# jianwen-xie/Latent-Space-Normalizing-Flow

Measured on AMD Instinct MI355X. Metric: latent-samples/sec through flow+logdet, nz=128 B=65536, higher is better.
Workload: dtype bf16x3; 1 GPU; CIFAR-10 flow prior nz=128 f_width=64 f_depth=5 affine, forward+logdet+log-prob, B=65536 synthetic z per evaluation (BASELINE.json configs[2]); rows_per_gpu=65536, global_rows=65536, parallelism=single GPU, streams=3, clock_ramp_launches_before_warmup=600

## Files before the change

### latent-space-normalizing-flow_amd/csrc/lsnf_device.h

```cpp
#pragma once
#include <hip/hip_runtime.h>
#include <type_traits>
#include "lsnf_layout.h"

typedef float f32x16 __attribute__((ext_vector_type(16)));
typedef float f32x4 __attribute__((ext_vector_type(4)));

#define LSNF_WG_THREADS 256
#define LSNF_WG_WAVES 4
#define LSNF_WG_SAMPLES (LSNF_WG_WAVES * 32)

#define LSNF_AS1 __attribute__((address_space(1)))
#define LSNF_AS3 __attribute__((address_space(3)))

static inline hipError_t lsnf_allow_big_lds(const void* kernel, unsigned long long* done_mask) {
    int dev = 0;
    hipError_t e = hipGetDevice(&dev);
    if (e != hipSuccess) return e;
    if (dev >= 0 && dev < 64 && ((*done_mask >> dev) & 1ull)) return hipSuccess;
    e = hipFuncSetAttribute(kernel, hipFuncAttributeMaxDynamicSharedMemorySize, 160 * 1024);
    if (e != hipSuccess) return e;
    if (dev >= 0 && dev < 64) *done_mask |= 1ull << dev;
    return hipSuccess;
}
// ... 25 lines not shown
    static constexpr int OFF_S4 = OFF_S3 + LSNF_FRAG_FLOATS * P3 * KT3;
    static constexpr int FWD_BLOCK = OFF_S4 + LSNF_FRAG_FLOATS * P4 * KT4;
    static constexpr int FWD_CONST = 32 * NP + 32;
    static constexpr int INV_BLOCK = LSNF_FRAG_FLOATS * NZT * NZT;
    static constexpr int INV_CONST = 32 * NZT;
    static constexpr int OFF_B4 = 0;
    static constexpr int OFF_B3 = OFF_B4 + LSNF_FRAG_FLOATS * WT * 2 * HT;
    static constexpr int OFF_B2 = OFF_B3 + LSNF_FRAG_FLOATS * WT * WT;
    static constexpr int OFF_B1 = OFF_B2 + LSNF_FRAG_FLOATS * HT * WT;
    static constexpr int BWD_BLOCK = OFF_B1 + LSNF_FRAG_FLOATS * NZT * NZT;
    static constexpr int MAXKT = (NZT > WT ? NZT : WT);
    static constexpr int SLOT = 2 * MAXKT * LSNF_FRAG_FLOATS;
};

#define LSNF_STATS_SLOTS 64
__device__ __forceinline__ void lsnf_publish_stats(double* stats, double sum_ll, double sum_logdet, int rows, int lane) {
    const unsigned grid = gridDim.x, wg = blockIdx.x;
    unsigned long long* ticket = reinterpret_cast<unsigned long long*>(&stats[2]);
    int last = 0;
    if (lane == 0) {
        const unsigned s = wg % LSNF_STATS_SLOTS;
        double* sub = stats + 8 + 4 * s;
        const double r0 = atomicAdd(&sub[0], sum_ll);
        const double r1 = atomicAdd(&sub[1], sum_logdet);
        unsigned long long inc = 1ull;
        asm volatile("" : "+v"(inc) : "v"(r0), "v"(r1));
        bool slot_done = true;
        if (grid > LSNF_STATS_SLOTS) {
            const unsigned long long n_s = (grid - s + LSNF_STATS_SLOTS - 1) / LSNF_STATS_SLOTS;
            unsigned long long* st = reinterpret_cast<unsigned long long*>(&sub[2]);
            slot_done = atomicAdd(st, inc) == n_s - 1;
            if (slot_done) atomicExch(st, 0ull);
            inc = 1ull;
        }
        if (slot_done) {
            const unsigned long long slots = grid > LSNF_STATS_SLOTS ? LSNF_STATS_SLOTS : grid;
            if (atomicAdd(ticket, inc) == slots - 1) { last = 1; atomicExch(ticket, 0ull); }
// ... 24 lines not shown
        if (PIECES % NW == 0 || seg < PIECES) {
            const float* g = gsrc + seg * 256 + lane * 4;
            float* l = lbuf + seg * 256;
            __builtin_amdgcn_global_load_lds((const LSNF_AS1 void*)g, (LSNF_AS3 void*)l, 16, 0, 0);
        }
    }
}

__device__ __forceinline__ void lsnf_panel_barrier() {
    asm volatile("s_waitcnt vmcnt(0)" ::: "memory");
#ifndef LSNF_ABLATE_BARRIER
    __syncthreads();
#endif
}

template <int KT>
__device__ __forceinline__ void lsnf_panel_mma(f32x16& acc, const f32x16* in, const float* lbuf, int lane) {
    const f32x4* wp = reinterpret_cast<const f32x4*>(lbuf) + lane;
    __builtin_amdgcn_sched_barrier(0);
    f32x4 w0 = wp[0], w1 = wp[64], w2 = wp[128], w3 = wp[192];
    __builtin_amdgcn_sched_group_barrier(0x100, 4, 0);
#pragma unroll
    for (int kt = 0; kt < KT; ++kt) {
        f32x4 n0 = w0, n1 = w1, n2 = w2, n3 = w3;
        if (kt + 1 < KT) {
            n0 = wp[((kt + 1) * 4 + 0) * 64]; n1 = wp[((kt + 1) * 4 + 1) * 64];
            n2 = wp[((kt + 1) * 4 + 2) * 64]; n3 = wp[((kt + 1) * 4 + 3) * 64];
        }
#define LSNF_MFMA4(W, G)                                                                      \
        acc = __builtin_amdgcn_mfma_f32_32x32x2f32(W[0], in[kt][4 * G + 0], acc, 0, 0, 0);    \
// ... 14 lines not shown
#pragma unroll
    for (int q = 0; q < 4; ++q) {
        const f32x4 v = b[q];
        a[4 * q + 0] = v[0]; a[4 * q + 1] = v[1]; a[4 * q + 2] = v[2]; a[4 * q + 3] = v[3];
    }
    return a;
}

__device__ __forceinline__ f32x16 lsnf_zero16() {
    f32x16 a;
#pragma unroll
    for (int r = 0; r < 16; ++r) a[r] = 0.0f;
    return a;
}

__device__ __forceinline__ f32x16 lsnf_relu16(f32x16 a) {
#pragma unroll
    for (int r = 0; r < 16; ++r) a[r] = fmaxf(a[r], 0.0f);
    return a;
}

__device__ __forceinline__ void lsnf_sigmoid_log2(float p, float& sig, float& l2) {
    const float pc = __builtin_amdgcn_fmed3f(p, -80.0f, 80.0f);
    const float e = __builtin_amdgcn_exp2f(pc * -1.4426950408889634f);
    const float d = 1.0f + e;
    sig = __builtin_amdgcn_rcpf(d);
    l2 = __builtin_amdgcn_logf(d);
}

__device__ __forceinline__ void lsnf_sigmoid_logsig(float p, float& sig, float& lsig) {
#ifdef LSNF_ABLATE_EPILOGUE
    sig = p * 0.25f + 0.5f; lsig = p; return;
#endif
// ... 251 lines not shown
```

### latent-space-normalizing-flow_amd/csrc/lsnf_fwd.hip

```cpp
#include <stdlib.h>
#include "lsnf_device.h"

namespace {

template <int HT_, int WT_>
struct FwdCfg : LsnfStackCfg<HT_, WT_> {
    using B = LsnfStackCfg<HT_, WT_>;
    static constexpr int BLOCK_FLOATS = B::FWD_BLOCK, CONST_FLOATS = B::FWD_CONST;
};

struct FwdArgs {
    const float* consts;
    const float* panels;
    const float* z_in;
    const float* objective;
    float* z_out;
    float* logdet_out;
    float* ll_out;
    float* z_saved;
    float* act_saved;
    int B, nz, half, n_blocks, vec4;
    double* stats;
    unsigned long long* stamps;
};
// ... 19 lines not shown
    constexpr int FWD_THREADS = 64 * FWD_WAVES;
    constexpr int HT = C::HT, WT = C::WT, NZT = C::NZT;
    extern __shared__ __attribute__((aligned(16))) float smem[];
    float* cst = smem;
    float* buf0 = smem + a.n_blocks * C::CONST_FLOATS;
    const int tid = threadIdx.x;
    const int wave = __builtin_amdgcn_readfirstlane(tid >> 6);
    const int lane = tid & 63;
    const int m = lane & 31, h = lane >> 5;

    LSNF_STAMP(0);
    LSNF_STAMP_RT(50);
    LsnfPipeT<FWD_WAVES> pipe;
    pipe.buf0 = buf0; pipe.slot = C::SLOT; pipe.wave = wave; pipe.lane = lane;
    pipe.template prime<lsnf_first_ktc(C::P1, C::KT1)>(a.panels);
    for (int i = tid; i < a.n_blocks * C::CONST_FLOATS; i += FWD_THREADS) cst[i] = a.consts[i];

    const long sample = ((long)blockIdx.x * FWD_WAVES + wave) * 32 + m;
    const bool live = sample < a.B;
    const long row = live ? sample : (long)a.B - 1;

    f32x16 x[NZT];
#ifdef LSNF_ABLATE_IO
#pragma unroll
    for (int t = 0; t < NZT; ++t)
#pragma unroll
        for (int r = 0; r < 16; ++r) x[t][r] = 0.001f * (float)(lane + r + t);
    float ell = 0.0f;
#else
    lsnf_load_rows<HT>(x, a.z_in, row, a.nz, a.half, h, a.vec4);
    float ell = a.objective ? a.objective[row] : 0.0f;
// ... 80 lines not shown
    if (live) {
        {
            float* zo = a.z_out + sample * (long)a.nz;
#pragma unroll
            for (int t = HT; t < NZT; ++t) lsnf_store_tile<HT>(t, x[t], zo, a.half, h, a.vec4);
        }
        if (h == 0) {
            a.logdet_out[sample] = ell;
            if (a.ll_out) a.ll_out[sample] = (-0.5f * ss + 1.8378770664093453f) + ell;
        }
    }
    if (a.stats) {
        float sl = (live && h == 0) ? ((-0.5f * ss + 1.8378770664093453f) + ell) : 0.0f;
        float sd = (live && h == 0) ? ell : 0.0f;
        double dl = (double)sl, dd = (double)sd;
#pragma unroll
        for (int o = 16; o > 0; o >>= 1) { dl += __shfl_xor(dl, o, 64); dd += __shfl_xor(dd, o, 64); }
        __syncthreads();
        double* red = reinterpret_cast<double*>(buf0);
        if (lane == 0) { red[2 * wave] = dl; red[2 * wave + 1] = dd; }
        __syncthreads();
        if (wave == 0) {
            double tl = 0.0, td = 0.0;
            for (int w = 0; w < FWD_WAVES; ++w) { tl += red[2 * w]; td += red[2 * w + 1]; }
            lsnf_publish_stats(a.stats, tl, td, a.B, lane);
        }
    }
    LSNF_STAMP(40);
    asm volatile("s_waitcnt vmcnt(0)" ::: "memory");
    LSNF_STAMP(41);
    LSNF_STAMP_RT(51);
}
// ... 40 lines not shown
```

### latent-space-normalizing-flow_amd/csrc/lsnf_fwd3.hip

```cpp
#include <stdlib.h>
#include "lsnf_l16.h"

namespace {



template <int HT_, int WT_>
struct Fwd3Cfg : LsnfStackCfg<HT_, WT_> {
    using S = LsnfStackCfg<HT_, WT_>;
    static constexpr int F = L16_FRAG_FLOATS;
    static constexpr int OFF3_S2 = F * S::P1 * S::KT1;
    static constexpr int OFF3_S3 = OFF3_S2 + F * S::P2 * S::KT2;
    static constexpr int OFF3_S4 = OFF3_S3 + F * S::P3 * S::KT3;
    static constexpr int BLOCK3 = OFF3_S4 + F * S::P4 * S::KT4;
    static constexpr int SLOT3 = 2 * S::MAXKT * F;
    static constexpr int CONST_FLOATS = S::FWD_CONST;
};

struct Fwd3Args {
    const float* consts; const float* panels3;
    const float* z_in; const float* objective;
    float* z_out; float* logdet_out; float* ll_out; float* z_saved; float* act_saved;
    int B, nz, half, n_blocks, vec4;
    double* stats;
// ... 49 lines not shown
    }
    bool bad = false;
#endif
    Pipe3<F3_WAVES> pipe;
    pipe.buf0 = buf0; pipe.slot = C::SLOT3; pipe.wave = wave; pipe.lane = lane;
    pipe.template prime<first_kib(C::P1, C::KT1)>(a.panels3);

    int sample[2], rows[2]; bool live[2];
#pragma unroll
    for (int st = 0; st < 2; ++st) { sample[st] = wbase + 16 * st + n; live[st] = sample[st] < a.B; rows[st] = live[st] ? sample[st] : a.B - 1; }

    f32x16 x[NZT];
#pragma unroll
    for (int t = 0; t < NZT; ++t) x[t] = l16_load_tile<HT>(t, a.z_in, rows, a.nz, a.half, g, a.vec4);
    __builtin_amdgcn_sched_barrier(0);
    for (int i = tid; i < a.n_blocks * C::CONST_FLOATS; i += THREADS) cst[i] = a.consts[i];
    float ell[2];
#pragma unroll
    for (int st = 0; st < 2; ++st) ell[st] = a.objective ? a.objective[rows[st]] : 0.0f;

    const LsnfActLayout al = lsnf_act_layout(a.B, HT, WT);
    const LsnfDumpLayout dl = lsnf_dump_layout(a.B, a.nz, a.width);
    const bool w4 = (a.width & 3) == 0;
    const size_t wtile = (size_t)blockIdx.x * F3_WAVES + wave;
    for (int blk = 0; blk < a.n_blocks; ++blk) {
        float* act = (a.act_saved && wtile * 32 < (size_t)a.B)
                         ? a.act_saved + (size_t)blk * al.per_block + wtile * al.per_tile : nullptr;
        const float* cb = cst + blk * C::CONST_FLOATS;
        const float* gblk = a.panels3 + (size_t)blk * C::BLOCK3;
        const bool more = blk + 1 < a.n_blocks;
        const float* gnext = more ? gblk + C::BLOCK3 : nullptr;
// ... 119 lines not shown
            int smp = sample[st];
            asm volatile("" : "+v"(smp));
            float ld = ell[st];
#if LSNF_L16_PARTS == 2
            if (wave_bad && st == 0 && n == 0) ld = __builtin_bit_cast(float, LSNF_F16_SENTINEL_BITS);
#endif
            a.logdet_out[smp] = ld;
            if (a.ll_out) a.ll_out[smp] = ll[st];
        }
    }
    if (a.stats) {
        double dl = 0.0, dd = 0.0;
#pragma unroll
        for (int st = 0; st < 2; ++st)
            if (live[st] && g == 0) { dl += (double)ll[st]; dd += (double)ell[st]; }
#pragma unroll
        for (int o = 8; o > 0; o >>= 1) { dl += __shfl_xor(dl, o, 64); dd += __shfl_xor(dd, o, 64); }
        __syncthreads();
        double* red = reinterpret_cast<double*>(buf0);
        if (lane == 0) { red[2 * wave] = dl; red[2 * wave + 1] = dd; }
        __syncthreads();
        if (wave == 0) {
            double tl = 0.0, td = 0.0;
            for (int w = 0; w < F3_WAVES; ++w) { tl += red[2 * w]; td += red[2 * w + 1]; }
            lsnf_publish_stats(a.stats, tl, td, a.B, lane);
        }
    }
    F3_STAMP(41, "s_memtime");
    F3_STAMP(51, "s_memrealtime");
}

template <class C>
// ... 58 lines not shown
```

### latent-space-normalizing-flow_amd/csrc/lsnf_fwd3p.hip

```cpp
#include <stdlib.h>
#include <type_traits>
#include "lsnf_l16.h"

#if LSNF_L16_PARTS != 3
#error "lsnf_fwd3p.hip is the three-term bf16 kernel"
#endif

#ifndef LSNF_FILLMASK
#define LSNF_FILLMASK 0x7f
#endif

namespace {

struct Fwd3pArgs {
    const float* consts; const float* panels3;
    const float* z_in; const float* objective;
    float* z_out; float* logdet_out; float* ll_out;
    int B, nz, half, n_blocks, vec4;
    double* stats;
    float* hdump; int width;
    float* z_saved; float* act_saved;
    unsigned long long* stamps;
};

// ... 5 lines not shown
         if (a.stamps && lane == 0) a.stamps[(((size_t)blockIdx.x * NWAVES + wave) & 2047) * 64 + (i)] = t_; } while (0)
#else
#define P_STAMP(i, INSN) do {} while (0)
#endif

template <int WT_>
struct Fwd3pCfg : LsnfStackCfg<2, WT_> {
    using S = LsnfStackCfg<2, WT_>;
    static constexpr int F = LSNF_FRAG3_FLOATS;
    static constexpr int OFF3_S2 = F * S::P1 * S::KT1;
    static constexpr int OFF3_S3 = OFF3_S2 + F * S::P2 * S::KT2;
    static constexpr int OFF3_S4 = OFF3_S3 + F * S::P3 * S::KT3;
    static constexpr int BLOCK3 = OFF3_S4 + F * S::P4 * S::KT4;
    static constexpr int SLOT3 = 2 * S::MAXKT * F;
    static constexpr int CONST_FLOATS = S::FWD_CONST;
};

__device__ __forceinline__ void keep(unsigned a, unsigned b, unsigned c) { asm volatile("" :: "v"(a), "v"(b), "v"(c)); }
__device__ __forceinline__ void keep(float a, float b, float c, float d, float e) { asm volatile("" :: "v"(a), "v"(b), "v"(c), "v"(d), "v"(e)); }

struct StepDesc { int acc, tile, s, frag; };
template <int KT> constexpr StepDesc mkstep(int acc, int tl, int in_tile, int kt, int s) { return StepDesc{acc, in_tile, s, ((tl * KT + kt) * 2 + s) * 3}; }

struct Tile16 { f32x4v q[4]; };
struct SplitTile16 { unsigned d[2][3][4]; };

template <int HT, int ST>
__device__ __forceinline__ Tile16 load_tile16(int t, const float* __restrict__ z, const int* rows, int nz, int half, int g, int vw) {
    Tile16 x;
    const int hh = t / HT, tt = t % HT;
// ... 54 lines not shown
    for (int j = 0; j < i; ++j)
        if (PH::at(j).acc == PH::at(i).acc && PH::at(j).s == PH::at(i).s) return false;
    return true;
}
template <int ST> __device__ __forceinline__ constexpr int unit_quad(int q) { return ST == 2 ? q : (q & ~1); }
template <int ST> __device__ __forceinline__ constexpr int unit_pair0(int q) { return ST == 2 ? 0 : (q & 1); }
template <int ST> __device__ __forceinline__ constexpr int unit_st(int q) { return ST == 2 ? (q & 1) : 0; }
template <bool RELU, int ST>
__device__ __forceinline__ void split_q16(const Tile16& x, int q, SplitTile16& out) {
#pragma clang fp contract(off)
    const int ft = q >> 1, st = unit_st<ST>(q), qr = unit_quad<ST>(q);
#pragma unroll
    for (int jj = 0; jj < ST; ++jj) {
        const int j = unit_pair0<ST>(q) + jj;
        float a = x.q[qr][2 * j], b = x.q[qr][2 * j + 1];
        if (RELU) { a = fmaxf(a, 0.0f); b = fmaxf(b, 0.0f); }
        const unsigned p1 = pk_bf16(a, b);
        a -= __builtin_bit_cast(float, p1 << 16); b -= __builtin_bit_cast(float, p1 & 0xffff0000u);
        const unsigned p2 = pk_bf16(a, b);
        a -= __builtin_bit_cast(float, p2 << 16); b -= __builtin_bit_cast(float, p2 & 0xffff0000u);
        const int d = 2 * ft + j;
        out.d[st][0][d] = p1; out.d[st][1][d] = p2; out.d[st][2][d] = pk_bf16(a, b);
        keep(out.d[st][0][d], out.d[st][1][d], out.d[st][2][d]);
    }
}
template <int ST>
__device__ __forceinline__ void sigmoid_q16(Tile16& p, int q, float* lsum ) {
    const int st = unit_st<ST>(q), qr = unit_quad<ST>(q), r0 = 2 * unit_pair0<ST>(q);
#pragma unroll
    for (int r = r0; r < r0 + 2 * ST; ++r) {
        float sig, l2;
// ... 31 lines not shown
    if (st) off += (unsigned)(16 * nz * 4);
    off = (32 * tt + 16 * ft + 4 * g < half) ? off : 0x80000000u;
    const u32x4s v = __builtin_bit_cast(u32x4s, x.q[q]);
    __builtin_amdgcn_raw_buffer_store_b128(v, rs.r[hh], off + (unsigned)((32 * tt + 16 * ft) * 4), 0, LSNF_STASH_AUX);
}
__device__ __forceinline__ void stash_sigma_quad(const StashRsrc& rs, const StashLane& sl, int t, int q, const Tile16& sg) {
    if constexpr (!(LSNF_STASH_PARTS & 2)) return;
    const int ft = q >> 1, st = q & 1;
    const u32x4s v = __builtin_bit_cast(u32x4s, sg.q[q]);
    __builtin_amdgcn_raw_buffer_store_b128(v, rs.r[t], sl.soff + (unsigned)((2 * ft * 64 + 16 * st) * 16), 0, LSNF_STASH_AUX);
}
__device__ __forceinline__ void mask_q16(const Tile16& h, int q, unsigned (&mk)[2][2]) {
    if constexpr (!(LSNF_STASH_PARTS & 1)) return;
    unsigned m = 0;
#pragma unroll
    for (int r = 3; r >= 0; --r) m = __builtin_amdgcn_alignbit(m, __builtin_bit_cast(unsigned, 0.0f - h.q[q][r]), 31);
    mk[q & 1][q >> 1] = m;
    asm volatile("" :: "v"(m));
}
__device__ __forceinline__ void stash_mask_words(const StashRsrc& rs, const StashLane& sl, int tile, const unsigned (&mk)[2][2]) {
    if constexpr (!(LSNF_STASH_PARTS & 1)) return;
    const unsigned w0 = mk[0][0] | (mk[0][1] << 8), w1 = mk[1][0] | (mk[1][1] << 8);
    unsigned x = ((w0 << 16) | w1) << sl.msh;
    x = lsnf_pair_or32(x);
    __builtin_amdgcn_raw_buffer_store_b32(x >> 16, rs.r[0], sl.moff + (unsigned)(tile * 64 * 4), 0, 0);
    __builtin_amdgcn_raw_buffer_store_b32(x & 0xffffu, rs.r[0], sl.moff + (unsigned)((tile * 64 + 16) * 4), 0, 0);
}
__device__ __forceinline__ void stash_h_quad(const StashRsrc& rs, const StashLane& sl, int t, int q, const Tile16& h, int width) {
    const int ft = q >> 1, st = q & 1;
    f32x4v r;
#pragma unroll
    for (int j = 0; j < 4; ++j) r[j] = fmaxf(h.q[q][j], 0.0f);
    const unsigned off = (32 * t + 16 * ft < width) ? sl.hoff : 0x80000000u;
    __builtin_amdgcn_raw_buffer_store_b128(__builtin_bit_cast(u32x4s, r), rs.r[t], off + (unsigned)((ft * 2 + st) * 1024), 0, LSNF_STASH_AUX);
}

template <int NM, int NV>
__device__ __forceinline__ void pin_mfma() {
    lsnf_static_for<NM>([&](auto mc) {
        constexpr int m = decltype(mc)::value, V = NV / NM + (m < NV % NM ? 1 : 0);
        __builtin_amdgcn_sched_group_barrier(0x008, 1, 0);
        if constexpr (V > 0) __builtin_amdgcn_sched_group_barrier(0x402, V, 0);
    });
}
template <class PH, int ST, class Fill, class Mid>
__device__ __forceinline__ void run_phase16(Tile16* acc, const float* bias_ptr , const SplitTile16* in, const float* lbuf, int lane, Fill&& fill, Mid&& mid) {
    const bf16x8* wp = reinterpret_cast<const bf16x8*>(lbuf) + lane;
// ... 119 lines not shown
    const int wave = __builtin_amdgcn_readfirstlane(tid >> 6);
    const int lane = tid & 63;
    const int n = lane & 15, g = lane >> 4;
    P_STAMP(0, "s_memtime");
    P_STAMP(50, "s_memrealtime");
    const int n_phases = 4 * a.n_blocks;
    auto phase_src = [&](int k) -> const float* {
        const float* gb = a.panels3 + (size_t)(k >> 2) * C::BLOCK3;
        const int j = k & 3;
        return gb + (j == 0 ? 0 : (j == 1 ? 2 * 4 * F : (j == 2 ? C::OFF3_S2 : C::OFF3_S4)));
    };
    auto sync_issue = [&](int k, auto left) {
#ifdef LSNF_ABL_SKIPSYNC
        if ((LSNF_ABL_SKIPSYNC >> (k & 3)) & 1) return;
#endif
        asm volatile("s_waitcnt vmcnt(%0)" :: "n"(decltype(left)::value) : "memory");
        __syncthreads();
#ifdef LSNF_FWD3Q_BURST_DMA
        if (k + 1 < n_phases) issue_kib<48, NWAVES>(phase_src(k + 1), buf0 + ((k + 1) & 1) * SLOT, wave, lane);
#endif
    };
    constexpr int PER_WAVE = 48 / NWAVES, EVERY = STASH ? 1 : 16 / PER_WAVE, LAST_DMA = (PER_WAVE - 1) * EVERY;
    using Left0 = std::integral_constant<int, 0>;
    using LeftS1a = std::integral_constant<int, stores_after<TS1a>(LAST_DMA)>;
    using LeftS1b = std::integral_constant<int, stores_after<TS1b>(LAST_DMA)>;
    using LeftS23 = std::integral_constant<int, stores_after<TS23>(LAST_DMA) + (STASH == 2 ? 1 : 0)>;
    using LeftS4 = std::integral_constant<int, stores_after<TS4>(LAST_DMA)>;
    const float* dma_src = nullptr; float* dma_dst = nullptr;
    auto dma_arm = [&](int k) {
        dma_src = phase_src(k + 1 < n_phases ? k + 1 : k);
        dma_dst = buf0 + ((k + 1) & 1) * SLOT;
    };
    auto dma_step = [&](auto ic) {
#ifndef LSNF_FWD3Q_BURST_DMA
        constexpr int i = decltype(ic)::value;
        if constexpr (i % EVERY == 0 && i / EVERY < PER_WAVE) issue_piece<NWAVES>(dma_src, dma_dst, i / EVERY, wave, lane);
#endif
    };
// ... 2 lines not shown
    int sample[2] = {0, 0}, rows[2] = {0, 0}; bool live[2] = {false, false};
#pragma unroll
    for (int st = 0; st < ST; ++st) { sample[st] = wbase + 16 * st + n; live[st] = sample[st] < a.B; rows[st] = live[st] ? sample[st] : a.B - 1; }

    Tile16 v[NZT];
    SplitTile16 xs[NZT];
    Tile16 p1, t1;
    float lsum[2] = {0.0f, 0.0f};
    {
        const Tile16 x0 = load_tile16<HT, ST>(0, a.z_in, rows, a.nz, a.half, g, a.vec4);
        const Tile16 x1 = load_tile16<HT, ST>(1, a.z_in, rows, a.nz, a.half, g, a.vec4);
        v[2] = load_tile16<HT, ST>(2, a.z_in, rows, a.nz, a.half, g, a.vec4);
        v[3] = load_tile16<HT, ST>(3, a.z_in, rows, a.nz, a.half, g, a.vec4);
        __builtin_amdgcn_sched_barrier(0);
        issue_kib<48, NWAVES>(phase_src(0), buf0, wave, lane);
        for (int i = tid; i < a.n_blocks * C::CONST_FLOATS; i += THREADS) cst[i] = a.consts[i];
#pragma unroll
        for (int q = 0; q < 4; ++q) { split_q16<false, ST>(x0, q, xs[0]); split_q16<false, ST>(x1, q, xs[1]); }
        split_q16<false, ST>(v[2], 0, xs[2]); split_q16<false, ST>(v[2], 1, xs[2]);
#pragma unroll
        for (int q = 0; q < 4; ++q)
#pragma unroll
            for (int r = 0; r < 4; ++r) { p1.q[q][r] = 80.0f; t1.q[q][r] = 0.0f; }
    }
    float ell[2];
#pragma unroll
    for (int st = 0; st < 2; ++st) ell[st] = (st < ST && a.objective) ? a.objective[rows[st]] : 0.0f;
    float ss01[2] = {0.0f, 0.0f};
    StashLane sl0 = {0u, 0u, 0u, 0u};
    const LsnfActLayout al = lsnf_act_layout(a.B, HT, WT);
    const unsigned zbytes = (unsigned)a.B * (unsigned)a.nz * 4u, abytes = (unsigned)(al.per_block * 4);
    if constexpr (STASH) {
        const unsigned tile_byte = (unsigned)(wbase >> 5) * (unsigned)(al.per_tile * 4), L = (unsigned)(n + 32 * (g & 1));
        sl0.zoff = ((unsigned)(wbase + n) * (unsigned)a.nz + 4u * g) * 4u;
        sl0.soff = tile_byte + ((unsigned)(g >> 1) * 64u + L) * 16u;
        sl0.moff = tile_byte + (unsigned)(al.mask_off * 4) + L * 4u;
        sl0.msh = 4u * (g >> 1);
        sl0.hoff = (unsigned)(wbase >> 5) * (unsigned)(32 * a.width * 4) + (unsigned)(n * 4 + g) * 16u;
    }
    const LsnfDumpLayout dl = lsnf_dump_layout(a.B, a.nz, a.width);
    const unsigned hbytes = (unsigned)(((size_t)a.B + 31) / 32 * 32 * a.width * 4);
    sync_issue(0, Left0{});
    P_STAMP(1, "s_memtime");

    for (int blk = 0; blk < a.n_blocks; ++blk) {
        const float* cb = cst + blk * C::CONST_FLOATS;
        const bool more = blk + 1 < a.n_blocks;
        const int k0 = 4 * blk;
        SplitTile16 vh[4];
        SplitTile16 h2s[WT];
        Tile16 hh[4], tp[4];
        const bool zs = STASH && a.z_saved != nullptr, as = STASH && a.act_saved != nullptr;
        const float* zc = more ? (zs ? a.z_saved + (size_t)blk * a.B * a.nz : a.z_out) : a.z_out;
        const float* zp = blk > 0 ? (zs ? a.z_saved + (size_t)(blk - 1) * a.B * a.nz : a.z_out) : a.z_out;
        const StashRsrc rs_zc = stash_rsrc(zc, (more && !zs) ? 0u : zbytes, (unsigned)a.half * 4u);
        const StashRsrc rs_zp = stash_rsrc(zp, (blk > 0 && !zs) ? 0u : zbytes, (unsigned)a.half * 4u);
        const StashRsrc rs_ac = stash_rsrc(as ? a.act_saved + (size_t)blk * al.per_block : a.z_out, as ? abytes : 0u, 4096u);
// ... 97 lines not shown
                    if constexpr (i == 8) stash_mask_words(rs_ac, sl, WT + 1, mk3);
                }
                if constexpr (STASH == 2 && i < 4) stash_h_quad(rs_h2, sl, 1, i, hh[3], a.width);
                if constexpr (i >= 9 && i < 13) { sigmoid_q16<ST>(tp[0], i - 9, lsum); if constexpr (STASH) stash_sigma_quad(rs_ac, sl, 0, i - 9, tp[0]); }
                if constexpr (i == 12) couple_q16<ST>(v[2], tp[1], tp[0], 0);
                if constexpr (i == 13) { couple_q16<ST>(v[2], tp[1], tp[0], 1); couple_q16<ST>(v[2], tp[1], tp[0], 2); couple_q16<ST>(v[2], tp[1], tp[0], 3); }
                if constexpr (i >= 14) split_q16<false, ST>(v[2], i - 14, xs[2]);
            }, dma_step);
            p1 = tp[2]; t1 = tp[3];
        }
        if (blk == 1) P_STAMP(14, "s_memtime");
    }
    P_STAMP(40, "s_memtime");
#pragma unroll
    for (int q = 0; q < 4; ++q) { sigmoid_q16<ST>(p1, q, lsum); couple_q16<ST>(v[3], t1, p1, q); }
    if constexpr (STASH) {
        const bool as = a.act_saved != nullptr;
        const StashRsrc rs_al = stash_rsrc(as ? a.act_saved + (size_t)(a.n_blocks - 1) * al.per_block : a.z_out, as ? abytes : 0u, 4096u);
#pragma unroll
        for (int q = 0; q < 4; ++q) stash_sigma_quad(rs_al, sl0, 1, q, p1);
    }
#pragma unroll
    for (int st = 0; st < ST; ++st) ell[st] = ell[st] + -0.6931471805599453f * l16_group_sum(lsum[st]);

    float ss[2] = {ss01[0], ss01[1]};
    int ln_e = lane;
    asm volatile("" : "+v"(ln_e));
    const int smp_e[2] = {wbase + (ln_e & 15), wbase + 16 + (ln_e & 15)};
#pragma unroll
    for (int t = HT; t < NZT; ++t) {
#pragma unroll
        for (int ft = 0; ft < 2; ++ft)
#pragma unroll
            for (int st = 0; st < ST; ++st)
#pragma unroll
                for (int r = 0; r < 4; ++r) ss[st] += v[t].q[2 * ft + st][r] * v[t].q[2 * ft + st][r];
        store_tile16<HT, ST>(t, v[t], a.z_out, smp_e, live, a.nz, a.half, g, a.vec4);
    }
    float ll[2] = {0.0f, 0.0f};
#pragma unroll
    for (int st = 0; st < ST; ++st) {
        ll[st] = (-0.5f * l16_group_sum(ss[st]) + 1.8378770664093453f) + ell[st];
        if (live[st] && g == 0) {
            const int smp = smp_e[st];
            a.logdet_out[smp] = ell[st];
            if (a.ll_out) a.ll_out[smp] = ll[st];
        }
    }
    asm volatile("s_waitcnt vmcnt(0)" ::: "memory");
    if (a.stats) {
        double dl = 0.0, dd = 0.0;
#pragma unroll
        for (int st = 0; st < ST; ++st)
            if (live[st] && g == 0) { dl += (double)ll[st]; dd += (double)ell[st]; }
#pragma unroll
        for (int o = 8; o > 0; o >>= 1) { dl += __shfl_xor(dl, o, 64); dd += __shfl_xor(dd, o, 64); }
        __syncthreads();
        double* red = reinterpret_cast<double*>(buf0);
        if (lane == 0) { red[2 * wave] = dl; red[2 * wave + 1] = dd; }
        __syncthreads();
        if (wave == 0) {
            double tl = 0.0, td = 0.0;
            for (int w = 0; w < NWAVES; ++w) { tl += red[2 * w]; td += red[2 * w + 1]; }
            lsnf_publish_stats(a.stats, tl, td, a.B, lane);
        }
    }
    P_STAMP(41, "s_memtime");
    P_STAMP(51, "s_memrealtime");
}

size_t fwd3q_lds(int n_blocks) {
// ... 51 lines not shown
```

### latent-space-normalizing-flow_amd/csrc/lsnf_small3.h

```cpp
#pragma once
#include "lsnf_device.h"

namespace {

typedef __bf16 bf16x2 __attribute__((ext_vector_type(2)));
typedef __bf16 bf16x8 __attribute__((ext_vector_type(8)));
typedef float f32x2v __attribute__((ext_vector_type(2)));
typedef unsigned u32x2 __attribute__((ext_vector_type(2)));

#define S3_SAMPLES 16
#define S3_BTILE_FLOATS 768

__device__ __forceinline__ unsigned pk_bf16(float a, float b) {
    const f32x2v v = {a, b};
    return __builtin_bit_cast(unsigned, __builtin_convertvector(v, bf16x2));
}
__device__ __forceinline__ void split4(const f32x4& x, u32x2* out ) {
#pragma clang fp contract(off)
#pragma unroll
    for (int q = 0; q < 2; ++q) {
        float a = x[2 * q], b = x[2 * q + 1];
        const unsigned p1 = pk_bf16(a, b);
        a -= __builtin_bit_cast(float, p1 << 16); b -= __builtin_bit_cast(float, p1 & 0xffff0000u);
        const unsigned p2 = pk_bf16(a, b);
// ... 83 lines not shown
        } else {
            __builtin_amdgcn_sched_group_barrier(0x008, REST - NL, 0);
        }
        __builtin_amdgcn_sched_barrier(0);
        b = nb;
    });
    if constexpr (EV > 0 && K1 == KT) epi(ST - 1);
}
template <int KT>
__device__ __forceinline__ void refill_last(UFrags<KT>& f, const bf16x8* r, int q) { f.w[KT - 1][q] = r[((KT - 1) * 6 + q) * 64]; }
__device__ __forceinline__ f32x4 unit_bias(const float* cst, int ft, int g) {
    return *reinterpret_cast<const f32x4*>(cst + (g & 1) * 16 + 4 * (2 * ft + (g >> 1)));
}
__device__ __forceinline__ f32x4 relu4(f32x4 a) {
#pragma unroll
    for (int r = 0; r < 4; ++r) a[r] = fmaxf(a[r], 0.0f);
    return a;
}
template <int HT>
__device__ __forceinline__ f32x4 load_row_half(int t, int ft, const float* __restrict__ zr, int half, int g, int vw) {
    const int hh = t / HT, tt = t % HT, f0 = 32 * tt + 16 * ft + 4 * g, col0 = hh * half + f0;
    f32x4 v = {0.f, 0.f, 0.f, 0.f};
    if (vw == 4) {
        if (f0 < half) v = *reinterpret_cast<const f32x4*>(zr + col0);
    } else if (vw == 2) {
        if (f0 < half) { const f32x2 a = *reinterpret_cast<const f32x2*>(zr + col0); v[0] = a[0]; v[1] = a[1]; }
        if (f0 + 2 < half) { const f32x2 a = *reinterpret_cast<const f32x2*>(zr + col0 + 2); v[2] = a[0]; v[3] = a[1]; }
    } else {
#pragma unroll
        for (int j = 0; j < 4; ++j) v[j] = (f0 + j < half) ? zr[col0 + j] : 0.0f;
    }
// ... 31 lines not shown
```

### latent-space-normalizing-flow_amd/csrc/lsnf_small3_fwd.hip

```cpp
#include <stdlib.h>
#include "lsnf_small3.h"

namespace {

template <int HT_, int WT_>
struct Small3Cfg : LsnfStackCfg<HT_, WT_> {
    using S = LsnfStackCfg<HT_, WT_>;
    static constexpr int F = LSNF_FRAG3_FLOATS;
    static constexpr int OFF3_S2 = F * S::P1 * S::KT1;
    static constexpr int OFF3_S3 = OFF3_S2 + F * S::P2 * S::KT2;
    static constexpr int OFF3_S4 = OFF3_S3 + F * S::P3 * S::KT3;
    static constexpr int BLOCK3 = OFF3_S4 + F * S::P4 * S::KT4;
    static constexpr int CONST_FLOATS = S::FWD_CONST;
    static constexpr int NU2 = (2 * WT_ + 3) / 4;
};
template <class C, int ST>
struct Small3Lds {
    static constexpr int XT = C::NZT * S3_BTILE_FLOATS;
    static constexpr int HL = C::WT * S3_BTILE_FLOATS;
    static constexpr int L_X = 0;
    static constexpr int L_H1 = L_X + ST * XT;
    static constexpr int L_H2 = L_H1 + ST * HL;
    static constexpr int L_RED = L_H2 + ST * HL;
    static constexpr int L_CONST = L_RED + ST * 4 * 16 * 2;
// ... 327 lines not shown
    if (wave == 0) {
        double dl = 0.0, dd = 0.0;
#pragma unroll
        for (int st = 0; st < ST; ++st) {
            float s2 = 0.0f, el = 0.0f;
#pragma unroll
            for (int w = 0; w < 4; ++w) { s2 += RED[((st * 4 + w) * 16 + n) * 2]; el += RED[((st * 4 + w) * 16 + n) * 2 + 1]; }
            const float ll = (-0.5f * s2 + 1.8378770664093453f) + el;
            if (live[st] && g == 0) {
                a.logdet_out[sample[st]] = el;
                if (a.ll_out) a.ll_out[sample[st]] = ll;
                dl += (double)ll; dd += (double)el;
            }
        }
        if (a.stats) {
#pragma unroll
            for (int o = 8; o > 0; o >>= 1) { dl += __shfl_xor(dl, o, 64); dd += __shfl_xor(dd, o, 64); }
            lsnf_publish_stats(a.stats, dl, dd, a.B, lane);
        }
    }
    S3_STAMP(41, "s_memtime");
    S3_STAMP(51, "s_memrealtime");
}

struct RestashArgs {
    const float* consts; const float* panels3b;
    const float* z_out; const float* z_saved; float* act_saved;
    int B, nz, half, depth, vec4;
};
template <class C>
__global__ __launch_bounds__(256, 1) void lsnf_small3_restash_kernel(const RestashArgs a) {
    constexpr int HT = C::HT, WT = C::WT, NU2 = C::NU2;
// ... 149 lines not shown
```

### latent-space-normalizing-flow_amd/csrc/lsnf_small_fwd.hip

```cpp
#include "lsnf_small.h"

namespace {

template <int HT_, int WT_>
struct SmallFwdCfg : LsnfStackCfg<HT_, WT_> {
    using S = LsnfStackCfg<HT_, WT_>;
    using S::HT; using S::WT; using S::NZT;
    static constexpr int BLOCK_FLOATS = S::FWD_BLOCK, CONST_FLOATS = S::FWD_CONST;
    using S1 = SmallStage<NZT, NZT>;
    using S2 = SmallStage<WT, HT>;
    using S3 = SmallStage<WT, WT>;
    using S4 = SmallStage<2 * HT, WT>;
    static constexpr int T_X = 0;
    static constexpr int T_V = T_X + 2 * NZT;
    static constexpr int T_H1 = T_V + S1::OUT_TILES;
    static constexpr int T_H2 = T_H1 + S2::OUT_TILES;
    static constexpr int T_TP = T_H2 + S3::OUT_TILES;
    static constexpr int T_END = T_TP + S4::OUT_TILES;
    static constexpr int AUX_FLOATS = 64 * (HT + NZT + 2);
};

struct SmallFwdArgs {
    const float* consts; const float* panels;
    const float* z_in; const float* objective;
// ... 142 lines not shown
        if (live) lsnf_store_tile<HT>(wave, x, a.z_out + sample * (long)a.nz, a.half, h, vec4);
    }
    __syncthreads();
    if (wave == 0) {
        float ss = 0.0f;
#pragma unroll
        for (int t = 0; t < NZT; ++t) ss += ssb[64 * t + lane];
        ss = lsnf_pair_sum(ss);
        const float ll = (-0.5f * ss + 1.8378770664093453f) + ell;
        if (live && h == 0) {
            a.logdet_out[sample] = ell;
            if (a.ll_out) a.ll_out[sample] = ll;
        }
        if (a.stats) {
            double dl = (live && h == 0) ? (double)ll : 0.0, dd = (live && h == 0) ? (double)ell : 0.0;
#pragma unroll
            for (int o = 16; o > 0; o >>= 1) { dl += __shfl_xor(dl, o, 64); dd += __shfl_xor(dd, o, 64); }
            lsnf_publish_stats(a.stats, dl, dd, a.B, lane);
        }
    }
    SMALL_STAMP(60);
}

template <class C>
size_t small_fwd_lds(int n_blocks) { return ((size_t)C::T_END * LSNF_TILE_FLOATS + C::AUX_FLOATS + (size_t)n_blocks * C::CONST_FLOATS) * sizeof(float); }

template <class C>
hipError_t launch_small_fwd(const SmallFwdArgs& a, hipStream_t stream) {
    const size_t lds = small_fwd_lds<C>(a.n_blocks);
    auto kern = lsnf_small_fwd_kernel<C>;
    static unsigned long long lds_ok = 0;
    if (hipError_t e = lsnf_allow_big_lds((const void*)kern, &lds_ok); e != hipSuccess) return e;
// ... 25 lines not shown
```

Before: 750.1 million latent-samples/s.

## Micro-optimize forward kernels: DPP reductions, buffer-load constants, integer ReLU, epilogue reorder

Replaces shuffle-based double reductions with DPP and permlane16_swap row sums. Copies the per-block constants into LDS with batched 128-bit buffer loads instead of a scalar strided loop. Computes ReLU as an integer max on the bit pattern. In fwd3p it moves the log-likelihood math ahead of the stash stores and waits for memory once, and it hides the stats offsets from scalar promotion. Each change trims instruction count or latency in prologue and epilogue code, at the cost of more complex code and behaviour for NaN and negative-zero inputs that may differ from fmaxf.

```diff
diff --git a/latent-space-normalizing-flow_amd/csrc/lsnf_device.h b/latent-space-normalizing-flow_amd/csrc/lsnf_device.h
--- a/latent-space-normalizing-flow_amd/csrc/lsnf_device.h
+++ b/latent-space-normalizing-flow_amd/csrc/lsnf_device.h
@@ -63,13 +63,35 @@
 };
 
 #define LSNF_STATS_SLOTS 64
+__device__ __forceinline__ double lsnf_row16_sum(double v) {
+#define LSNF_DPP_ADD(CTRL)                                                                                        \
+    {   const unsigned long long u = __builtin_bit_cast(unsigned long long, v);                                   \
+        const unsigned lo = (unsigned)__builtin_amdgcn_update_dpp(0, (int)(unsigned)u, CTRL, 0xf, 0xf, false);    \
+        const unsigned hi = (unsigned)__builtin_amdgcn_update_dpp(0, (int)(unsigned)(u >> 32), CTRL, 0xf, 0xf, false); \
+        v += __builtin_bit_cast(double, ((unsigned long long)hi << 32) | lo); }
+    LSNF_DPP_ADD(0xB1)
+    LSNF_DPP_ADD(0x4E)
+    LSNF_DPP_ADD(0x141)
+    LSNF_DPP_ADD(0x140)
+#undef LSNF_DPP_ADD
+    return v;
+}
+__device__ __forceinline__ double lsnf_half32_sum(double v) {
+    const unsigned long long u = __builtin_bit_cast(unsigned long long, lsnf_row16_sum(v));
+    const auto lo = __builtin_amdgcn_permlane16_swap((unsigned)u, (unsigned)u, false, false);
+    const auto hi = __builtin_amdgcn_permlane16_swap((unsigned)(u >> 32), (unsigned)(u >> 32), false, false);
+    return __builtin_bit_cast(double, ((unsigned long long)(unsigned)hi[0] << 32) | (unsigned)lo[0]) +
+           __builtin_bit_cast(double, ((unsigned long long)(unsigned)hi[1] << 32) | (unsigned)lo[1]);
+}
 __device__ __forceinline__ void lsnf_publish_stats(double* stats, double sum_ll, double sum_logdet, int rows, int lane) {
     const unsigned grid = gridDim.x, wg = blockIdx.x;
-    unsigned long long* ticket = reinterpret_cast<unsigned long long*>(&stats[2]);
     int last = 0;
     if (lane == 0) {
         const unsigned s = wg % LSNF_STATS_SLOTS;
-        double* sub = stats + 8 + 4 * s;
+        unsigned sub_at = 8 + 4 * s, ticket_at = 2;
+        asm volatile("" : "+v"(sub_at), "+v"(ticket_at));
+        double* sub = stats + sub_at;
+        unsigned long long* ticket = reinterpret_cast<unsigned long long*>(stats + ticket_at);
         const double r0 = atomicAdd(&sub[0], sum_ll);
         const double r1 = atomicAdd(&sub[1], sum_logdet);
         unsigned long long inc = 1ull;
@@ -124,6 +146,24 @@
 #endif
 }
 
+#define LSNF_WAIT_VMCNT0() __builtin_amdgcn_s_waitcnt(0x0F70)
+
+template <int THREADS, int MAX_VEC4>
+__device__ __forceinline__ void lsnf_consts_to_lds(float* cst, const float* src, int n_vec4, int tid) {
+    constexpr int PER_THREAD = (MAX_VEC4 + THREADS - 1) / THREADS;
+    typedef unsigned lsnf_u32x4 __attribute__((ext_vector_type(4)));
+    const __amdgpu_buffer_rsrc_t rs = __builtin_amdgcn_make_buffer_rsrc(const_cast<float*>(src), 0, n_vec4 * 16, 0x00020000);
+    lsnf_u32x4 c[PER_THREAD];
+#pragma unroll
+    for (int k = 0; k < PER_THREAD; ++k) c[k] = __builtin_amdgcn_raw_buffer_load_b128(rs, (tid + k * THREADS) * 16, 0, 0);
+    __builtin_amdgcn_sched_barrier(0);
+    LSNF_WAIT_VMCNT0();
+    __builtin_amdgcn_sched_barrier(0);
+#pragma unroll
+    for (int k = 0; k < PER_THREAD; ++k)
+        if (tid + k * THREADS < n_vec4) reinterpret_cast<lsnf_u32x4*>(cst)[tid + k * THREADS] = c[k];
+}
+
 template <int KT>
 __device__ __forceinline__ void lsnf_panel_mma(f32x16& acc, const f32x16* in, const float* lbuf, int lane) {
     const f32x4* wp = reinterpret_cast<const f32x4*>(lbuf) + lane;
@@ -168,9 +208,14 @@
     return a;
 }
 
+__device__ __forceinline__ float lsnf_relu(float x) {
+    const int b = __builtin_bit_cast(int, x);
+    return __builtin_bit_cast(float, b > 0 ? b : 0);
+}
+
 __device__ __forceinline__ f32x16 lsnf_relu16(f32x16 a) {
 #pragma unroll
-    for (int r = 0; r < 16; ++r) a[r] = fmaxf(a[r], 0.0f);
+    for (int r = 0; r < 16; ++r) a[r] = lsnf_relu(a[r]);
     return a;
 }
 
diff --git a/latent-space-normalizing-flow_amd/csrc/lsnf_fwd.hip b/latent-space-normalizing-flow_amd/csrc/lsnf_fwd.hip
--- a/latent-space-normalizing-flow_amd/csrc/lsnf_fwd.hip
+++ b/latent-space-normalizing-flow_amd/csrc/lsnf_fwd.hip
@@ -57,7 +57,9 @@
     LsnfPipeT<FWD_WAVES> pipe;
     pipe.buf0 = buf0; pipe.slot = C::SLOT; pipe.wave = wave; pipe.lane = lane;
     pipe.template prime<lsnf_first_ktc(C::P1, C::KT1)>(a.panels);
-    for (int i = tid; i < a.n_blocks * C::CONST_FLOATS; i += FWD_THREADS) cst[i] = a.consts[i];
+    static_assert(C::CONST_FLOATS % 4 == 0, "the constant blocks are copied in 16-byte groups");
+    for (int v0 = 0, n4 = a.n_blocks * (C::CONST_FLOATS / 4); v0 < n4; v0 += 8 * FWD_THREADS)
+        lsnf_consts_to_lds<FWD_THREADS, 8 * FWD_THREADS>(cst + 4 * v0, a.consts + 4 * v0, n4 - v0, tid);
 
     const long sample = ((long)blockIdx.x * FWD_WAVES + wave) * 32 + m;
     const bool live = sample < a.B;
@@ -168,8 +170,7 @@
         float sl = (live && h == 0) ? ((-0.5f * ss + 1.8378770664093453f) + ell) : 0.0f;
         float sd = (live && h == 0) ? ell : 0.0f;
         double dl = (double)sl, dd = (double)sd;
-#pragma unroll
-        for (int o = 16; o > 0; o >>= 1) { dl += __shfl_xor(dl, o, 64); dd += __shfl_xor(dd, o, 64); }
+        dl = lsnf_half32_sum(dl); dd = lsnf_half32_sum(dd);
         __syncthreads();
         double* red = reinterpret_cast<double*>(buf0);
         if (lane == 0) { red[2 * wave] = dl; red[2 * wave + 1] = dd; }
diff --git a/latent-space-normalizing-flow_amd/csrc/lsnf_fwd3.hip b/latent-space-normalizing-flow_amd/csrc/lsnf_fwd3.hip
--- a/latent-space-normalizing-flow_amd/csrc/lsnf_fwd3.hip
+++ b/latent-space-normalizing-flow_amd/csrc/lsnf_fwd3.hip
@@ -87,7 +87,9 @@
 #pragma unroll
     for (int t = 0; t < NZT; ++t) x[t] = l16_load_tile<HT>(t, a.z_in, rows, a.nz, a.half, g, a.vec4);
     __builtin_amdgcn_sched_barrier(0);
-    for (int i = tid; i < a.n_blocks * C::CONST_FLOATS; i += THREADS) cst[i] = a.consts[i];
+    static_assert(C::CONST_FLOATS % 4 == 0, "the constant blocks are copied in 16-byte groups");
+    for (int v0 = 0, n4 = a.n_blocks * (C::CONST_FLOATS / 4); v0 < n4; v0 += 8 * THREADS)
+        lsnf_consts_to_lds<THREADS, 8 * THREADS>(cst + 4 * v0, a.consts + 4 * v0, n4 - v0, tid);
     float ell[2];
 #pragma unroll
     for (int st = 0; st < 2; ++st) ell[st] = a.objective ? a.objective[rows[st]] : 0.0f;
@@ -237,8 +239,7 @@
 #pragma unroll
         for (int st = 0; st < 2; ++st)
             if (live[st] && g == 0) { dl += (double)ll[st]; dd += (double)ell[st]; }
-#pragma unroll
-        for (int o = 8; o > 0; o >>= 1) { dl += __shfl_xor(dl, o, 64); dd += __shfl_xor(dd, o, 64); }
+        dl = lsnf_row16_sum(dl); dd = lsnf_row16_sum(dd);
         __syncthreads();
         double* red = reinterpret_cast<double*>(buf0);
         if (lane == 0) { red[2 * wave] = dl; red[2 * wave + 1] = dd; }
diff --git a/latent-space-normalizing-flow_amd/csrc/lsnf_fwd3p.hip b/latent-space-normalizing-flow_amd/csrc/lsnf_fwd3p.hip
--- a/latent-space-normalizing-flow_amd/csrc/lsnf_fwd3p.hip
+++ b/latent-space-normalizing-flow_amd/csrc/lsnf_fwd3p.hip
@@ -43,6 +43,9 @@
     static constexpr int BLOCK3 = OFF3_S4 + F * S::P4 * S::KT4;
     static constexpr int SLOT3 = 2 * S::MAXKT * F;
     static constexpr int CONST_FLOATS = S::FWD_CONST;
+    static constexpr int LDS_FLOATS = 160 * 1024 / 4;
+    static constexpr int MAX_BLOCKS = (LDS_FLOATS - 2 * SLOT3) / CONST_FLOATS;
+    static_assert(CONST_FLOATS % 4 == 0, "the constant blocks are copied in 16-byte groups");
 };
 
 __device__ __forceinline__ void keep(unsigned a, unsigned b, unsigned c) { asm volatile("" :: "v"(a), "v"(b), "v"(c)); }
@@ -127,7 +130,7 @@
     for (int jj = 0; jj < ST; ++jj) {
         const int j = unit_pair0<ST>(q) + jj;
         float a = x.q[qr][2 * j], b = x.q[qr][2 * j + 1];
-        if (RELU) { a = fmaxf(a, 0.0f); b = fmaxf(b, 0.0f); }
+        if (RELU) { a = lsnf_relu(a); b = lsnf_relu(b); }
         const unsigned p1 = pk_bf16(a, b);
         a -= __builtin_bit_cast(float, p1 << 16); b -= __builtin_bit_cast(float, p1 & 0xffff0000u);
         const unsigned p2 = pk_bf16(a, b);
@@ -189,7 +192,7 @@
     if constexpr (!(LSNF_STASH_PARTS & 1)) return;
     unsigned m = 0;
 #pragma unroll
-    for (int r = 3; r >= 0; --r) m = __builtin_amdgcn_alignbit(m, __builtin_bit_cast(unsigned, 0.0f - h.q[q][r]), 31);
+    for (int r = 3; r >= 0; --r) m = __builtin_amdgcn_alignbit(m, 0u - __builtin_bit_cast(unsigned, lsnf_relu(h.q[q][r])), 31);
     mk[q & 1][q >> 1] = m;
     asm volatile("" :: "v"(m));
 }
@@ -205,7 +208,7 @@
     const int ft = q >> 1, st = q & 1;
     f32x4v r;
 #pragma unroll
-    for (int j = 0; j < 4; ++j) r[j] = fmaxf(h.q[q][j], 0.0f);
+    for (int j = 0; j < 4; ++j) r[j] = lsnf_relu(h.q[q][j]);
     const unsigned off = (32 * t + 16 * ft < width) ? sl.hoff : 0x80000000u;
     __builtin_amdgcn_raw_buffer_store_b128(__builtin_bit_cast(u32x4s, r), rs.r[t], off + (unsigned)((ft * 2 + st) * 1024), 0, LSNF_STASH_AUX);
 }
@@ -355,14 +358,14 @@
 #ifdef LSNF_ABL_SKIPSYNC
         if ((LSNF_ABL_SKIPSYNC >> (k & 3)) & 1) return;
 #endif
-        asm volatile("s_waitcnt vmcnt(%0)" :: "n"(decltype(left)::value) : "memory");
+        if constexpr (decltype(left)::value >= 0) asm volatile("s_waitcnt vmcnt(%0)" :: "n"(decltype(left)::value) : "memory");
         __syncthreads();
 #ifdef LSNF_FWD3Q_BURST_DMA
         if (k + 1 < n_phases) issue_kib<48, NWAVES>(phase_src(k + 1), buf0 + ((k + 1) & 1) * SLOT, wave, lane);
 #endif
     };
     constexpr int PER_WAVE = 48 / NWAVES, EVERY = STASH ? 1 : 16 / PER_WAVE, LAST_DMA = (PER_WAVE - 1) * EVERY;
-    using Left0 = std::integral_constant<int, 0>;
+    using LeftWaited = std::integral_constant<int, -1>;
     using LeftS1a = std::integral_constant<int, stores_after<TS1a>(LAST_DMA)>;
     using LeftS1b = std::integral_constant<int, stores_after<TS1b>(LAST_DMA)>;
     using LeftS23 = std::integral_constant<int, stores_after<TS23>(LAST_DMA) + (STASH == 2 ? 1 : 0)>;
@@ -395,7 +398,7 @@
         v[3] = load_tile16<HT, ST>(3, a.z_in, rows, a.nz, a.half, g, a.vec4);
         __builtin_amdgcn_sched_barrier(0);
         issue_kib<48, NWAVES>(phase_src(0), buf0, wave, lane);
-        for (int i = tid; i < a.n_blocks * C::CONST_FLOATS; i += THREADS) cst[i] = a.consts[i];
+        lsnf_consts_to_lds<THREADS, C::MAX_BLOCKS * (C::CONST_FLOATS / 4)>(cst, a.consts, a.n_blocks * (C::CONST_FLOATS / 4), tid);
 #pragma unroll
         for (int q = 0; q < 4; ++q) { split_q16<false, ST>(x0, q, xs[0]); split_q16<false, ST>(x1, q, xs[1]); }
         split_q16<false, ST>(v[2], 0, xs[2]); split_q16<false, ST>(v[2], 1, xs[2]);
@@ -421,7 +424,7 @@
     }
     const LsnfDumpLayout dl = lsnf_dump_layout(a.B, a.nz, a.width);
     const unsigned hbytes = (unsigned)(((size_t)a.B + 31) / 32 * 32 * a.width * 4);
-    sync_issue(0, Left0{});
+    sync_issue(0, LeftWaited{});
     P_STAMP(1, "s_memtime");
 
     for (int blk = 0; blk < a.n_blocks; ++blk) {
@@ -549,47 +552,48 @@
     P_STAMP(40, "s_memtime");
 #pragma unroll
     for (int q = 0; q < 4; ++q) { sigmoid_q16<ST>(p1, q, lsum); couple_q16<ST>(v[3], t1, p1, q); }
+#pragma unroll
+    for (int st = 0; st < ST; ++st) ell[st] = ell[st] + -0.6931471805599453f * l16_group_sum(lsum[st]);
+
+    float ss[2] = {ss01[0], ss01[1]};
+#pragma unroll
+    for (int t = HT; t < NZT; ++t)
+#pragma unroll
+        for (int ft = 0; ft < 2; ++ft)
+#pragma unroll
+            for (int st = 0; st < ST; ++st)
+#pragma unroll
+                for (int r = 0; r < 4; ++r) ss[st] += v[t].q[2 * ft + st][r] * v[t].q[2 * ft + st][r];
+    float ll[2] = {0.0f, 0.0f};
+#pragma unroll
+    for (int st = 0; st < ST; ++st) ll[st] = (-0.5f * l16_group_sum(ss[st]) + 1.8378770664093453f) + ell[st];
+    __builtin_amdgcn_sched_barrier(0);
+    LSNF_WAIT_VMCNT0();
+    __builtin_amdgcn_sched_barrier(0);
     if constexpr (STASH) {
         const bool as = a.act_saved != nullptr;
         const StashRsrc rs_al = stash_rsrc(as ? a.act_saved + (size_t)(a.n_blocks - 1) * al.per_block : a.z_out, as ? abytes : 0u, 4096u);
 #pragma unroll
         for (int q = 0; q < 4; ++q) stash_sigma_quad(rs_al, sl0, 1, q, p1);
     }
-#pragma unroll
-    for (int st = 0; st < ST; ++st) ell[st] = ell[st] + -0.6931471805599453f * l16_group_sum(lsum[st]);
-
-    float ss[2] = {ss01[0], ss01[1]};
     int ln_e = lane;
     asm volatile("" : "+v"(ln_e));
     const int smp_e[2] = {wbase + (ln_e & 15), wbase + 16 + (ln_e & 15)};
 #pragma unroll
-    for (int t = HT; t < NZT; ++t) {
-#pragma unroll
-        for (int ft = 0; ft < 2; ++ft)
-#pragma unroll
-            for (int st = 0; st < ST; ++st)
-#pragma unroll
-                for (int r = 0; r < 4; ++r) ss[st] += v[t].q[2 * ft + st][r] * v[t].q[2 * ft + st][r];
-        store_tile16<HT, ST>(t, v[t], a.z_out, smp_e, live, a.nz, a.half, g, a.vec4);
-    }
-    float ll[2] = {0.0f, 0.0f};
-#pragma unroll
-    for (int st = 0; st < ST; ++st) {
-        ll[st] = (-0.5f * l16_group_sum(ss[st]) + 1.8378770664093453f) + ell[st];
+    for (int t = HT; t < NZT; ++t) store_tile16<HT, ST>(t, v[t], a.z_out, smp_e, live, a.nz, a.half, g, a.vec4);
+#pragma unroll
+    for (int st = 0; st < ST; ++st)
         if (live[st] && g == 0) {
             const int smp = smp_e[st];
             a.logdet_out[smp] = ell[st];
             if (a.ll_out) a.ll_out[smp] = ll[st];
         }
-    }
-    asm volatile("s_waitcnt vmcnt(0)" ::: "memory");
     if (a.stats) {
         double dl = 0.0, dd = 0.0;
 #pragma unroll
         for (int st = 0; st < ST; ++st)
             if (live[st] && g == 0) { dl += (double)ll[st]; dd += (double)ell[st]; }
-#pragma unroll
-        for (int o = 8; o > 0; o >>= 1) { dl += __shfl_xor(dl, o, 64); dd += __shfl_xor(dd, o, 64); }
+        dl = lsnf_row16_sum(dl); dd = lsnf_row16_sum(dd);
         __syncthreads();
         double* red = reinterpret_cast<double*>(buf0);
         if (lane == 0) { red[2 * wave] = dl; red[2 * wave + 1] = dd; }
diff --git a/latent-space-normalizing-flow_amd/csrc/lsnf_small3.h b/latent-space-normalizing-flow_amd/csrc/lsnf_small3.h
--- a/latent-space-normalizing-flow_amd/csrc/lsnf_small3.h
+++ b/latent-space-normalizing-flow_amd/csrc/lsnf_small3.h
@@ -121,7 +121,7 @@
 }
 __device__ __forceinline__ f32x4 relu4(f32x4 a) {
 #pragma unroll
-    for (int r = 0; r < 4; ++r) a[r] = fmaxf(a[r], 0.0f);
+    for (int r = 0; r < 4; ++r) a[r] = lsnf_relu(a[r]);
     return a;
 }
 template <int HT>
diff --git a/latent-space-normalizing-flow_amd/csrc/lsnf_small3_fwd.hip b/latent-space-normalizing-flow_amd/csrc/lsnf_small3_fwd.hip
--- a/latent-space-normalizing-flow_amd/csrc/lsnf_small3_fwd.hip
+++ b/latent-space-normalizing-flow_amd/csrc/lsnf_small3_fwd.hip
@@ -365,8 +365,7 @@
             }
         }
         if (a.stats) {
-#pragma unroll
-            for (int o = 8; o > 0; o >>= 1) { dl += __shfl_xor(dl, o, 64); dd += __shfl_xor(dd, o, 64); }
+            dl = lsnf_row16_sum(dl); dd = lsnf_row16_sum(dd);
             lsnf_publish_stats(a.stats, dl, dd, a.B, lane);
         }
     }
diff --git a/latent-space-normalizing-flow_amd/csrc/lsnf_small_fwd.hip b/latent-space-normalizing-flow_amd/csrc/lsnf_small_fwd.hip
--- a/latent-space-normalizing-flow_amd/csrc/lsnf_small_fwd.hip
+++ b/latent-space-normalizing-flow_amd/csrc/lsnf_small_fwd.hip
@@ -180,8 +180,7 @@
         }
         if (a.stats) {
             double dl = (live && h == 0) ? (double)ll : 0.0, dd = (live && h == 0) ? (double)ell : 0.0;
-#pragma unroll
-            for (int o = 16; o > 0; o >>= 1) { dl += __shfl_xor(dl, o, 64); dd += __shfl_xor(dd, o, 64); }
+            dl = lsnf_half32_sum(dl); dd = lsnf_half32_sum(dd);
             lsnf_publish_stats(a.stats, dl, dd, a.B, lane);
         }
     }
```

After: 755.6 million latent-samples/s (median of 6 runs). Within noise of the previous version (+0.7%).
